# Sara-H-dev/Semantic_Segmentation_Of_StyleGAN2_Artifacts

Measured on AMD Instinct MI355X. Metric: training images/sec at 1024^2 bs=8 per GPU (MS-UNet Swin-T, fwd+DynamicLoss+bwd+AdamW), higher is better.
Workload: dtype bf16; 1 GPU; 1xMI355X 1024x1024 bs=8 Swin-T MS-UNet train step; model=MS-UNet swin_t, global_batch=8, world_size=1, img_size=1024, parallelism=dp1, grad_allreduce=f32, dead_branches=executed (no grad), step_execution=eager, params=42881040

## Files before the change

### include/msunet_hip.h

```cpp
#ifndef MSUNET_HIP_H
#define MSUNET_HIP_H

#ifdef __cplusplus
extern "C" {
#endif

int msu_layernorm_fwd(int dtype, int mode, const void* x, const void* b, const float* bscale,
                      long rows_per_sample, void* s_out, const float* gamma, const float* beta,
                      void* y, float* mean, float* rstd, long rows, int C, int H, int W, int Cin,
                      float eps, void* stream);
int msu_layernorm_bwd(int dtype, int mode, const void* dy, const void* x, const void* dres,
                      const float* gamma, const float* mean, const float* rstd, void* dx,
                      void* db, const float* bscale, long rows_per_sample, float* part,
                      int nparts, float* dgamma, float* dbeta, long rows, int C, int H, int W,
                      int Cin, int accumulate, void* stream);
int msu_layernorm_bwd3(int dtype, int mode, const void* dy, const void* x, const void* dres,
                       const void* dres2, const void* dres3, const float* gamma, const float* mean,
                       const float* rstd, void* dx, void* db, const float* bscale, long rows_per_sample,
                       float* part, int nparts, float* dgamma, float* dbeta, long rows, int C, int H, int W,
                       int Cin, int accumulate, void* stream);
int msu_ln_part_blocks(long rows, int C);
int msu_colsum_batch(int nseg, const float* const* part, const long* stride, const int* nparts, const int* n,
                     float* const* out, int accumulate, void* stream);
int msu_tail_reduce_mode(int mode);
// ... 46 lines not shown
int msu_conv3x3_wgrad(int dtype, int in_mode, const void* X, const void* dY, float* dW, float* db,
                      float* workspace, void* unused, int nchunk, int B, int H, int W, int Cin,
                      int Cout, void* stream);
int msu_conv3x3_wgrad2(int dtype, int in_mode, const void* X, const void* dY, float* dW, float* db,
                       float* workspace, int nchunk, int B, int H, int W, int Cin, int Cout, int accumulate,
                       void* stream);

int msu_win_attn_qkv_supported(int C, int nh);
int msu_win_attn_qkv_fwd(int dtype, const void* x, const void* w_qkv, const float* b_qkv, const float* table,
                         void* out, void* qkv_out, void* keep, float* workspace, int B, int H, int W, int C, int nh,
                         int shift, float p_drop, unsigned long long seed, const unsigned long long* seed_dev,
                         void* stream);
int msu_win_attn_qkv_fwd2(int dtype, const void* x, const void* w_qkv, const float* b_qkv, const float* table,
                          const void* w_proj, const float* b_proj, void* out, void* o_out, void* qkv_out, void* keep,
                          float* workspace, int B, int H, int W, int C, int nh, int shift, float p_drop,
                          unsigned long long seed, const unsigned long long* seed_dev, void* stream);

int msu_wgrad_splits(long M, int N, int K);
long msu_wgrad_workspace(long M, int N, int K);
int msu_linear_wgrad(int dtype, const void* dY, const void* X, float* dW, float* db, float* workspace,
                     long M, int N, int K, int accumulate, void* stream);
int msu_linear_wgrad_ld(int dtype, const void* dY, const void* X, float* dW, long ldw, float* db,
                        float* workspace, long M, int N, int K, int accumulate, void* stream);

int msu_linear_bwd_supported(long M, int K, int N);
long msu_linear_bwd_workspace(long M, int K, int N);
int msu_linear_bwd(int dtype, const void* dY, const void* X, const void* Wt, const void* H, void* dX, float* dW,
                   float* db, float* workspace, long M, int K, int N, int accumulate, void* stream);

int msu_tok_gemm_supported(long M, int N, int K);
int msu_tok_gemm_supported_epi(long M, int N, int K, int epi);
int msu_tok_gemm(int dtype, const void* A, const void* A2, int K1, const void* W, const float* bias, void* Y,
                 void* Y2, const void* H, long M, int N, int K, int epi, void* stream);
int msu_tok_gemm_plan(long M, int N, int K, long* out6);
int msu_nt_gemm_supported(long M, int N, int K);
int msu_nt_gemm_plan(long M, int N);
int msu_nt_gemm_mode(int mode);
int msu_nt_gemm(int dtype, const void* A, const void* W, const float* bias, void* Y, void* Y2, const void* H,
                long M, int N, int K, int epi, void* stream);
int msu_nt_gemm_cat(int dtype, const void* A, const void* A2, int K1, const void* W, const float* bias, void* Y,
                    long M, int N, int K, void* stream);
int msu_nt_gemm_kn(int dtype, const void* A, const void* Wk, const float* bias, void* Y, void* Y2, const void* H,
                   long M, int N, int K, int epi, void* stream);

int msu_mlp_fused_supported(int C, int Hd);
int msu_add_ln_mlp_fwd(int dtype, const void* a, const void* br, const float* bscale, long rows_per_sample,
// ... 64 lines not shown
```

### semantic_segmentation_of_stylegan2_artifacts_amd/_lib.py

```python
import ctypes
import os

from . import switches

_HERE = os.path.dirname(os.path.abspath(__file__))
LIB_PATH = switches.get("MSU_LIB_OVERRIDE") or os.path.join(_HERE, "libmsunet_hip.so")

P = ctypes.c_void_p
I = ctypes.c_int
L = ctypes.c_long
F = ctypes.c_float
D = ctypes.c_double
U64 = ctypes.c_ulonglong

SIGNATURES = {
    "msu_ln_part_blocks": (I, [L, I]),
    "msu_layernorm_fwd": (I, [I, I, P, P, P, L, P, P, P, P, P, P, L, I, I, I, I, F, P]),
    "msu_layernorm_bwd": (I, [I, I, P, P, P, P, P, P, P, P, P, L, P, I, P, P, L, I, I, I, I, I, P]),
    "msu_layernorm_bwd3": (I, [I, I, P, P, P, P, P, P, P, P, P, P, P, L, P, I, P, P, L, I, I, I, I, I, P]),
    "msu_reduce_rows": (I, [P, I, I, L, P, I, P]),
    "msu_tail_reduce_mode": (I, [I]),
    "msu_conv_mode": (I, [I]),
    "msu_head_fwd": (I, [I, P, P, P, P, P, P, P, L, I, F, P]),
    "msu_head_bwd": (I, [I, P, P, P, P, P, P, P, P, P, I, P, P, P, L, I, P]),
# ... 23 lines not shown
    "msu_dynloss_fwd2": (I, [I, P, P, I, L, F, F, F, P, I, P, P, P, P]),
    "msu_dynloss_fwd3": (I, [I, P, P, I, L, F, F, F, P, I, P, P, P, P, P]),
    "msu_dynloss_bwd2": (I, [I, P, P, P, P, P, I, L, F, F, F, P, P]),
    "msu_adamw": (I, [P, P, P, P, L, F, F, F, F, F, I, P, P, P]),
    "msu_nonfinite": (I, [P, L, P, P]),
    "msu_nonfinite2": (I, [P, L, P, L, P, P]),
    "msu_adamw_dev": (I, [P, P, P, P, L, P, D, D, D, D, P, P, P]),
    "msu_adamw_dev2": (I, [P, P, P, P, L, P, D, D, D, D, P, P, P, I, I, P]),
    "msu_step_advance": (I, [P, P, P]),
    "msu_cast": (I, [I, P, P, L, P]),
    "msu_colsum_batch": (I, [I, P, P, P, P, P, I, P]),
    "msu_conv3x3_weight": (I, [I, P, P, I, I, I, P]),
    "msu_transpose16_multi": (I, [P, P, P, I, I, P]),
    "msu_conv3x3_fwd": (I, [I, I, P, P, P, P, I, I, I, I, I, P]),
    "msu_conv3x3_fwd2": (I, [I, I, P, P, P, P, P, I, I, I, I, I, P]),
    "msu_conv3x3_dgrad": (I, [I, I, P, P, P, P, I, I, I, I, I, P]),
    "msu_conv3x3_wgrad_workspace": (L, [I, I, I, I, I]),
    "msu_conv3x3_wgrad": (I, [I, I, P, P, P, P, P, P, I, I, I, I, I, I, P]),
    "msu_conv3x3_wgrad2": (I, [I, I, P, P, P, P, P, I, I, I, I, I, I, I, P]),
    "msu_wgrad_splits": (I, [L, I, I]),
    "msu_wgrad_workspace": (L, [L, I, I]),
    "msu_linear_wgrad": (I, [I, P, P, P, P, P, L, I, I, I, P]),
    "msu_linear_wgrad_ld": (I, [I, P, P, P, L, P, P, L, I, I, I, P]),
    "msu_linear_bwd_supported": (I, [L, I, I]),
    "msu_linear_bwd_workspace": (L, [L, I, I]),
    "msu_linear_bwd": (I, [I, P, P, P, P, P, P, P, P, L, I, I, I, P]),
    "msu_tok_gemm_supported": (I, [L, I, I]),
    "msu_tok_gemm_supported_epi": (I, [L, I, I, I]),
    "msu_tok_gemm": (I, [I, P, P, I, P, P, P, P, P, L, I, I, I, P]),
    "msu_tok_gemm_plan": (I, [L, I, I, P]),
    "msu_nt_gemm_supported": (I, [L, I, I]),
    "msu_nt_gemm_plan": (I, [L, I]),
    "msu_nt_gemm_mode": (I, [I]),
    "msu_nt_gemm": (I, [I, P, P, P, P, P, P, L, I, I, I, P]),
    "msu_nt_gemm_kn": (I, [I, P, P, P, P, P, P, L, I, I, I, P]),
    "msu_nt_gemm_cat": (I, [I, P, P, I, P, P, P, L, I, I, P]),
    "msu_metrics_nblk": (I, [L]),
    "msu_seg_metrics": (I, [I, P, P, I, L, F, P, I, P, P]),
    "msu_augment_batch": (I, [P, P, P, P, P, P, I, I, I, P]),
    "msu_pred_maps_nblk": (I, [I, I]),
    "msu_pred_maps": (I, [I, P, P, P, I, I, I, F, F, F, F, I, I, P, P, P, P, P, P, P, P]),
}

_lib = None


# ... 35 lines not shown
```

### semantic_segmentation_of_stylegan2_artifacts_amd/csrc/common.h

```cpp
#pragma once
#include <hip/hip_runtime.h>
#include <hip/hip_bf16.h>
#include <stdint.h>

#include <mutex>

#define MSU_DEV __device__ __forceinline__

typedef __bf16 bf16x8 __attribute__((ext_vector_type(8)));
typedef float f32x4 __attribute__((ext_vector_type(4)));
typedef float f32x16 __attribute__((ext_vector_type(16)));
typedef uint32_t u32x4 __attribute__((ext_vector_type(4)));
typedef uint32_t u32x2 __attribute__((ext_vector_type(2)));
typedef float f32x2 __attribute__((ext_vector_type(2)));
typedef uint16_t bf16_t;
typedef _Float16 f16_t;
typedef _Float16 f16x8 __attribute__((ext_vector_type(8)));

enum MsuDtype { MSU_F32 = 0, MSU_BF16 = 1, MSU_F16 = 2 };

MSU_DEV float to_f32(float v) { return v; }
MSU_DEV float to_f32(bf16_t v) { return __uint_as_float(((uint32_t)v) << 16); }
template <typename T> MSU_DEV T from_f32(float v);
template <> MSU_DEV float from_f32<float>(float v) { return v; }
// ... 112 lines not shown
  const float cdf = 0.5f * (1.0f + erf_fast(x * 0.70710678118654752f, e));
  return fmaf(x * 0.39894228040143268f, e, cdf);
}

MSU_DEV f32x2 pk_fma(f32x2 a, f32x2 b, f32x2 c) { return __builtin_elementwise_fma(a, b, c); }
MSU_DEV f32x2 splat2(float v) { return f32x2{v, v}; }
MSU_DEV f32x2 erf_fast2(f32x2 x, f32x2& e_neg_x2) {
  const f32x2 ax = {fabsf(x.x), fabsf(x.y)};
  const f32x2 d = pk_fma(splat2(0.3275911f), ax, splat2(1.0f));
  const f32x2 t = {__builtin_amdgcn_rcpf(d.x), __builtin_amdgcn_rcpf(d.y)};
  f32x2 p = pk_fma(splat2(1.061405429f), t, splat2(-1.453152027f));
  p = pk_fma(p, t, splat2(1.421413741f));
  p = pk_fma(p, t, splat2(-0.284496736f));
  p = pk_fma(p, t, splat2(0.254829592f)) * t;
  const f32x2 q = -ax * ax;
  e_neg_x2 = f32x2{__expf(q.x), __expf(q.y)};
  const f32x2 r = pk_fma(-p, e_neg_x2, splat2(1.0f));
  return f32x2{copysignf(r.x, x.x), copysignf(r.y, x.y)};
}
MSU_DEV f32x2 gelu_fast2(f32x2 x) {
  f32x2 e;
  return splat2(0.5f) * x * (splat2(1.0f) + erf_fast2(x * splat2(0.70710678118654752f), e));
}

MSU_DEV float hash_uniform(uint64_t seed, uint64_t idx) {
  uint64_t z = seed + 0x9E3779B97F4A7C15ull * (idx + 1);
  z = (z ^ (z >> 30)) * 0xBF58476D1CE4E5B9ull;
  z = (z ^ (z >> 27)) * 0x94D049BB133111EBull;
  z ^= z >> 31;
  return (float)(uint32_t)(z >> 40) * (1.0f / 16777216.0f);
}

MSU_DEV uint64_t launch_seed(uint64_t seed, const unsigned long long* seed_dev) {
  if (seed_dev == nullptr) return seed;
  uint64_t z = seed ^ ((uint64_t)seed_dev[0] * 0x9E3779B97F4A7C15ull);
  z = (z ^ (z >> 31)) * 0xBF58476D1CE4E5B9ull;
  return z ^ (z >> 29);
}

MSU_DEV uint32_t fmix32_hash(uint32_t seed, uint32_t idx) {
  uint32_t x = idx * 0x9E3779B9u + seed;
  x ^= x >> 16; x *= 0x85EBCA6Bu;
  x ^= x >> 13; x *= 0xC2B2AE35u;
  return x ^ (x >> 16);
}
MSU_DEV uint32_t drop_thresh16(float p) { return (uint32_t)ceilf(p * 65536.0f); }
// ... 125 lines not shown
```

### semantic_segmentation_of_stylegan2_artifacts_amd/csrc/gemm_linbwd.hip

```cpp
#include <utility>

#include "common.h"
#include "reduce.h"

#ifndef MSU_EXP
#define MSU_EXP 0
#endif

namespace {

#ifndef MSU_LB_TS64
#define MSU_LB_TS64 1
#endif
constexpr int ts_of(int K, int N) { return (MSU_LB_TS64 && K == 96 && (N == 288 || N == 96)) ? 64 : 32; }
constexpr int NW = 8;
constexpr int NTHR = 64 * NW;

typedef short v4s __attribute__((ext_vector_type(4)));
typedef __attribute__((address_space(3))) v4s lds_v4s;

template <int I> using IC = std::integral_constant<int, I>;

template <typename F, int... I>
MSU_DEV __attribute__((always_inline)) void static_for_impl(F&& f, std::integer_sequence<int, I...>) {
// ... 82 lines not shown
MSU_DEV int wg_tile(int w, int i) {
  using P = Plan<K, N>;
  constexpr auto t = P::make();
  int jt = -1;
#pragma unroll
  for (int ww = 0; ww < NW; ++ww)
    if (w == ww && i < t.count[ww]) jt = t.tile[ww][i];
  return jt;
}

template <typename T, int K, int N, bool GG, bool GX = false>
__global__ void __launch_bounds__(NTHR, 1)
linbwd_kernel(const bf16_t* __restrict__ dY, const bf16_t* __restrict__ X, const bf16_t* __restrict__ Wt,
              const bf16_t* __restrict__ H, bf16_t* __restrict__ dX, float* __restrict__ part, long M) {
  using P = Plan<K, N>;
  constexpr int TM = ts_of(K, N);
  static_assert(!GG || TM == 32, "the GELU' operands are staged for 32-token steps");
  constexpr int LDW = N + 8, LDY = N + 8, LDX = ldx_of<K>();
  constexpr int CY = N / 8, CX = K / 8;
  constexpr int CHUNKS = TM * (CY + CX);
  constexpr int PER = (CHUNKS + NTHR - 1) / NTHR;
  constexpr int STAGE = TM * (LDY + LDX);
  constexpr int KT = P::KT, NS16 = P::NS16, DMAX = P::DMAX, WMAX = P::WMAX;
  extern __shared__ __attribute__((aligned(16))) unsigned char smem_raw[];
  bf16_t* sW = reinterpret_cast<bf16_t*>(smem_raw);
  bf16_t* sS = sW + K * LDW;
  const int tid = threadIdx.x, lane = tid & 63;
  const int wave = __builtin_amdgcn_readfirstlane(tid >> 6);
  const int h = lane >> 5;
  const long ntiles = (M + TM - 1) / TM;
  const int G = gridDim.x;
  const int b = blockIdx.x;
  const long nsteps = (ntiles - 1 - b) / G + 1;

  for (int i = tid; i < K * CY; i += NTHR) {
    const int r = i / CY, c = i - r * CY;
    *reinterpret_cast<u32x4*>(sW + r * LDW + 8 * c) = *reinterpret_cast<const u32x4*>(Wt + (long)r * N + 8 * c);
  }

  constexpr int D = ring_depth<K, N, GG>();
  u32x4 st[D][PER];
  int goff[PER], loff[PER];
#pragma unroll
  for (int j = 0; j < PER; ++j) {
    const int c = tid + NTHR * j;
    goff[j] = 0;
    loff[j] = 0;
    if (c < TM * CY) {
      const int r = c / CY, cc = c - r * CY;
      goff[j] = r * N + 8 * cc;
      loff[j] = r * LDY + 8 * cc;
    } else if (c < CHUNKS) {
      const int c2 = c - TM * CY;
      const int r = c2 / CX, cc = c2 - r * CX;
      goff[j] = r * K + 8 * cc;
      loff[j] = TM * LDY + r * LDX + 8 * cc;
    }
  }
  auto kind = [&](int j) __attribute__((always_inline)) {
    const int cw = wave * 64 + NTHR * j;
    return cw < TM * CY ? 0 : cw < CHUNKS ? 1 : 2;
  };
  auto load = [&](long step_, auto SET) __attribute__((always_inline)) {
    constexpr int set = decltype(SET)::value;
    const long step = step_ < nsteps ? step_ : nsteps - 1;
    const long m0 = (b + step * G) * TM;
    if (m0 + TM <= M) {
#pragma unroll
      for (int j = 0; j < PER; ++j) {
        const int kd = kind(j);
        const bf16_t* base = kd == 0 ? dY + m0 * N : kd == 1 ? X + m0 * K : dY;
        if constexpr ((MSU_EXP & 8) != 0) st[set][j] = u32x4{(unsigned)goff[j], 0u, 0u, 0u};
        else st[set][j] = gload16_s(base, 2u * (unsigned)goff[j]);
      }
    } else {
      const int t0 = opaque(tid);
#pragma unroll
      for (int j = 0; j < PER; ++j) {
        const int c = t0 + NTHR * j;
        const bf16_t* src = dY;
        if (c < TM * CY) {
          const int r = c / CY, cc = c - r * CY;
          const long m = m0 + r < M ? m0 + r : M - 1;
          src = dY + m * N + 8 * cc;
        } else if (c < CHUNKS) {
          const int c2 = c - TM * CY;
          const int r = c2 / CX, cc = c2 - r * CX;
          const long m = m0 + r < M ? m0 + r : M - 1;
          src = X + m * K + 8 * cc;
        }
        st[set][j] = gload16(src);
      }
    }
  };
  auto store = [&](long step, auto SET) __attribute__((always_inline)) {
    constexpr int set = decltype(SET)::value;
    if constexpr (GX) {
#pragma unroll
      for (int j = 0; j < PER; ++j) {
        if (kind(j) == 1) {
          u32x4& q = st[set][j];
#pragma unroll
          for (int i = 0; i < 4; ++i)
            q[i] = pack2<T>(gelu_fast(Fmt16<T>::lo(q[i])), gelu_fast(Fmt16<T>::hi(q[i])));
        }
      }
    }
    bf16_t* y = sS + (int)(step & 1) * STAGE;
    const long m0 = (b + step * G) * TM;
    if (m0 + TM <= M) {
#pragma unroll
      for (int j = 0; j < PER; ++j)
        if (kind(j) != 2) *reinterpret_cast<u32x4*>(y + loff[j]) = st[set][j];
    } else {
      const int t0 = opaque(tid);
#pragma unroll
      for (int j = 0; j < PER; ++j) {
        const int c = t0 + NTHR * j;
        const int r = c < TM * CY ? c / CY : (c - TM * CY) / CX;
        const u32x4 z = {0u, 0u, 0u, 0u};
        if (kind(j) != 2) *reinterpret_cast<u32x4*>(y + loff[j]) = m0 + r < M ? st[set][j] : z;
      }
    }
  };

  f32x16 accw[WMAX];
#pragma unroll
  for (int i = 0; i < WMAX; ++i) accw[i] = f32x16{0};
  constexpr int NP = N / 2, RG = NTHR / NP < TM ? NTHR / NP : TM;
  const int bp = tid % NP, bg = tid / NP;
  float db0 = 0.f, db1 = 0.f;

  static_for<D>([&](auto I) __attribute__((always_inline)) {
    load(decltype(I)::value, I);
  });
  store(0, IC<0>{});
  __syncthreads();

  auto body = [&](long s, auto SLOT) __attribute__((always_inline)) {
    constexpr int slot = decltype(SLOT)::value;
    const bf16_t* y = sS + (int)(s & 1) * STAGE;
    const bf16_t* x = y + TM * LDY;
    const long m0 = (b + s * G) * TM;
    u32x4 hv[DMAX][2];
    if constexpr (GG) {
      const long m = m0 + (lane & 31);
      const long mh = m < M ? m : M - 1;
#pragma unroll
      for (int d = 0; d < DMAX; ++d) {
        const int kt0 = wave + NW * d;
        if (MSU_LB_HALL || kt0 < KT) {
          const int kt = kt0 < KT ? kt0 : wave;
#pragma unroll
          for (int pp = 0; pp < 2; ++pp) hv[d][pp] = gload16(H + mh * K + 32 * kt + 16 * pp + 8 * h);
        }
      }
    }
    load(s + D, SLOT);

#pragma unroll
    for (int i = 0; i < WMAX; ++i) {
      const int jt = wg_tile<K, N>(wave, i);
      if (jt >= 0 && (MSU_EXP & 4) == 0) {
        const int jo = opaque(jt);
        const int kt = jo / P::NT, nt = jo - (jo / P::NT) * P::NT;
#pragma unroll
        for (int ks = 0; ks < TM / 16; ++ks)
          accw[i] = Fmt16<T>::mma32(frag_tr(x, LDX, 16 * ks, 32 * kt, lane), frag_tr(y, LDY, 16 * ks, 32 * nt, lane),
// ... 12 lines not shown

#pragma unroll
    for (int d = 0; d < DMAX; ++d) {
      const int kt = wave + NW * d;
#pragma unroll
      for (int tt = 0; tt < TM / 32; ++tt) if (kt < KT) {
        const long m = m0 + 32 * tt + (lane & 31);
        f32x16 acc = f32x16{0};
#pragma unroll 3
        for (int ns = 0; ns < ((MSU_EXP & 2) ? 0 : NS16); ++ns)
          acc = Fmt16<T>::mma32(frag_rows(sW, LDW, 32 * kt, 16 * ns, lane), frag_rows(y, LDY, 32 * tt, 16 * ns, lane),
                                acc);
#pragma unroll
        for (int pp = 0; pp < 2; ++pp) {
          const int g0 = 2 * pp;
          float v[8];
#pragma unroll
          for (int e = 0; e < 4; ++e) {
            const auto r = __builtin_amdgcn_permlane32_swap(__float_as_uint(acc[4 * g0 + e]),
                                                            __float_as_uint(acc[4 * g0 + 4 + e]), false, false);
            v[e] = __uint_as_float(r[0]);
            v[4 + e] = __uint_as_float(r[1]);
          }
          if constexpr (GG) {
#pragma unroll
            for (int e = 0; e < 4; ++e) {
              v[2 * e] *= gelu_grad_fast(Fmt16<T>::lo(hv[d][pp][e]));
              v[2 * e + 1] *= gelu_grad_fast(Fmt16<T>::hi(hv[d][pp][e]));
            }
          }
          const u32x4 pk = {pack2<T>(v[0], v[1]), pack2<T>(v[2], v[3]), pack2<T>(v[4], v[5]), pack2<T>(v[6], v[7])};
          if (m < M && (MSU_EXP & 1) == 0) *reinterpret_cast<u32x4*>(dX + m * K + 32 * kt + 16 * pp + 8 * h) = pk;
        }
      }
    }
    if (s + 1 < nsteps) {
      store(s + 1, IC<(slot + 1) % D>{});
    }
    __syncthreads();
  };
  for (long s = 0; s < nsteps; s += D) {
    static_for<D>([&](auto I) __attribute__((always_inline)) {
      if (s + decltype(I)::value < nsteps) body(s + decltype(I)::value, I);
    });
  }

  float* pw = part + (long)b * (N * K + N);
// ... 112 lines not shown
```

### semantic_segmentation_of_stylegan2_artifacts_amd/csrc/gemm_wgrad.hip

```cpp
#include <stdlib.h>

#include "common.h"
#include "mfma_frag.h"
#include "reduce.h"

#ifndef MSU_EXP
#define MSU_EXP 0
#endif

namespace {

constexpr int BM = 64;

MSU_DEV void unpack8(const u32x4& q, float (&v)[8]) {
#pragma unroll
  for (int i = 0; i < 4; ++i) {
    v[2 * i] = __uint_as_float(q[i] << 16);
    v[2 * i + 1] = __uint_as_float(q[i] & 0xffff0000u);
  }
}

template <typename T, int NTW>
__global__ void __launch_bounds__(256) wgrad_kernel(const T* __restrict__ dY, const T* __restrict__ X,
                                                    float* __restrict__ part, float* __restrict__ dbpart,
                                                    long M, int N, int K, long mchunk) {
  constexpr int WT = 16 * NTW;
  constexpr int BT = 2 * WT;
  constexpr int LDT = BT + 8;
  constexpr int EPC = 16 / (int)sizeof(T);
  constexpr int CPR = BT / EPC;
  constexpr int CH = BM * CPR / 256;
  __shared__ __attribute__((aligned(16))) T sA[2][BM * LDT];
  __shared__ __attribute__((aligned(16))) T sB[2][BM * LDT];
  const int tid = threadIdx.x, lane = tid & 63, wave = tid >> 6;
  const int ntk = (K + BT - 1) / BT;
  const int tn = blockIdx.x / ntk, tk = blockIdx.x - (blockIdx.x / ntk) * ntk;
  const int n0 = tn * BT, k0 = tk * BT;
  const long m_begin = (long)blockIdx.y * mchunk;
  long m_end = m_begin + mchunk;
  if (m_end > M) m_end = M;
  const int wn = (wave >> 1) * WT, wk = (wave & 1) * WT;

  f32x4 acc[NTW][NTW];
#pragma unroll
  for (int i = 0; i < NTW; ++i)
#pragma unroll
    for (int j = 0; j < NTW; ++j) acc[i][j] = f32x4{0.f, 0.f, 0.f, 0.f};
  float dbacc = 0.f;
  const bool do_bias = dbpart != nullptr && tk == 0;

  uint4 ra[CH], rb[CH];
  auto load_regs = [&](long m0) {
#pragma unroll
    for (int c = 0; c < CH; ++c) {
      const int idx = tid + 256 * c;
      const int r = idx / CPR, col = (idx - r * CPR) * EPC;
      const long m = m0 + r;
      const bool ok = m < m_end;
      ra[c] = (ok && n0 + col < N) ? *reinterpret_cast<const uint4*>(dY + m * (long)N + n0 + col) : make_uint4(0, 0, 0, 0);
      rb[c] = (ok && k0 + col < K) ? *reinterpret_cast<const uint4*>(X + m * (long)K + k0 + col) : make_uint4(0, 0, 0, 0);
    }
  };
  auto store_regs = [&](int buf) {
#pragma unroll
    for (int c = 0; c < CH; ++c) {
      const int idx = tid + 256 * c;
      const int r = idx / CPR, col = (idx - r * CPR) * EPC;
      *reinterpret_cast<uint4*>(&sA[buf][r * LDT + col]) = ra[c];
      *reinterpret_cast<uint4*>(&sB[buf][r * LDT + col]) = rb[c];
    }
  };

  int buf = 0;
  if (m_begin < m_end) {
    load_regs(m_begin);
    store_regs(0);
  }
  __syncthreads();
  for (long m0 = m_begin; m0 < m_end; m0 += BM) {
    const bool more = m0 + BM < m_end;
    if (more) load_regs(m0 + BM);
    const T* A = sA[buf];
    const T* B = sB[buf];
    auto rowA = [&](int k) { return A + k * LDT; };
    auto rowB = [&](int k) { return B + k * LDT; };
#pragma unroll
    for (int ks = 0; ks < BM; ks += 32)
#pragma unroll
      for (int i = 0; i < NTW; ++i)
#pragma unroll
        for (int j = 0; j < NTW; ++j) TR<T>::mma(acc[i][j], rowA, wn + 16 * i, rowB, wk + 16 * j, ks, lane);
// ... 1 lines not shown
#pragma unroll 8
      for (int r = 0; r < BM; ++r) dbacc += to_f32(A[r * LDT + tid]);
    }
    if (more) store_regs(buf ^ 1);
    __syncthreads();
    buf ^= 1;
  }
  float* out = part + (long)blockIdx.y * N * K;
#pragma unroll
  for (int i = 0; i < NTW; ++i)
#pragma unroll
    for (int j = 0; j < NTW; ++j)
#pragma unroll
      for (int r = 0; r < 4; ++r) {
        const int n = n0 + wn + 16 * i + (lane >> 4) * 4 + r;
        const int k = k0 + wk + 16 * j + (lane & 15);
        if (n < N && k < K) out[(long)n * K + k] = acc[i][j][r];
      }
  if (do_bias && tid < BT && n0 + tid < N) dbpart[(long)blockIdx.y * N + n0 + tid] = dbacc;
}

template <int WN, int WK> constexpr int wgrad_nw() { return WN * WK == 3 ? 3 : 4; }

template <typename T, int NTW, int WN, int WK, int NST>
__global__ void __launch_bounds__(256) wgrad_wave_kernel(const bf16_t* __restrict__ dY, const bf16_t* __restrict__ X,
                                                         float* __restrict__ part, float* __restrict__ dbpart,
                                                         long M, int N, int K, long mchunk, int ntiles) {
  constexpr int NW = wgrad_nw<WN, WK>();
  constexpr int WM = NW / (WN * WK), WT = 16 * NTW, BN = WN * WT, BK = WK * WT, RS = 32 * WM;
  static_assert(WM * WN * WK == NW, "wave split");
  constexpr int SA = (BN + 8) / 8, SB = (BK + 8) / 8;
  constexpr int LA = 8 * SA, LB = 8 * SB;
  constexpr int SLOTS = RS * (SA + SB);
  constexpr int INS = ((SLOTS + 63) / 64 + NW - 1) / NW * NW;
  constexpr int PER_WAVE = INS / NW;
  constexpr int STG = INS * 64 * 8;
  static_assert(NST >= 2 && PER_WAVE * (NST - 2) < 64, "vmcnt");
  extern __shared__ __attribute__((aligned(16))) unsigned char smem_raw[];
  bf16_t* lds = reinterpret_cast<bf16_t*>(smem_raw);
  const int tid = threadIdx.x, lane = tid & 63;
  const int wave = __builtin_amdgcn_readfirstlane(tid >> 6);
  const int wni = wave % WN, wki = (wave / WN) % WK, wmi = wave / (WN * WK);
  const int ntk = K / BK;
  const int item = xcd_remap(blockIdx.x, gridDim.x);
  const int split = item / ntiles, tile = item - split * ntiles;
  const int tn = tile / ntk, tk = tile - (tile / ntk) * ntk;
  const int n0 = tn * BN, k0 = tk * BK;
// ... 34 lines not shown
    }
  };

  f32x4 acc[NTW][NTW];
  f32x4 accb[NTW];
#pragma unroll
  for (int i = 0; i < NTW; ++i) {
    accb[i] = f32x4{0.f, 0.f, 0.f, 0.f};
#pragma unroll
    for (int j = 0; j < NTW; ++j) acc[i][j] = f32x4{0.f, 0.f, 0.f, 0.f};
  }
  const bool do_bias = dbpart != nullptr && tk == 0 && wki == 0;
  const bf16x8 ones = splat8<T>(1.0f, 1.0f, 1.0f);
  const int q = (lane & 15) >> 2, p4 = 4 * (lane & 3), r0 = wmi * 32 + 2 * (4 * ((lane >> 4) & 1) + q) + (lane >> 5);
  const int laneA = r0 * LA + wni * WT + p4, laneB = RS * LA + r0 * LB + wki * WT + p4;
  auto tr8 = [](const bf16_t* p, int second) {
    typedef __attribute__((address_space(3))) msu_v4s lds_v4s;
    const msu_v4s lo = __builtin_amdgcn_ds_read_tr16_b64_v4i16((lds_v4s*)(p));
    const msu_v4s hi = __builtin_amdgcn_ds_read_tr16_b64_v4i16((lds_v4s*)(p + second));
    msu_v4s both[2] = {lo, hi};
    return *reinterpret_cast<bf16x8*>(both);
  };

#pragma unroll
  for (int st = 0; st < NST - 1; ++st) issue(st);
  for (int st = 0; st < nstage; ++st) {
    wait_vmcnt<PER_WAVE * (NST - 2)>();
    __builtin_amdgcn_s_barrier();
    issue(st + NST - 1);
    if constexpr (MSU_EXP & 2) continue;
    const bf16_t* buf = lds + (st % NST) * STG;
    const uint32_t pa = lds_u32(buf + laneA), pb = lds_u32(buf + laneB);
    bf16x8 bf[NTW], af[2];
    unroll_for<NTW>([&](auto J) {
      constexpr int j = decltype(J)::value;
      bf[j] = tr8_untracked<32 * j, 32 * j + 32 * LB>(pb);
    });
    af[0] = tr8_untracked<0, 32 * LA>(pa);
    asm volatile("s_waitcnt lgkmcnt(0)" ::: "memory");
#pragma unroll
    for (int j = 0; j < NTW; ++j) asm volatile("" : "+v"(bf[j]));
    asm volatile("" : "+v"(af[0]));
    unroll_for<NTW>([&](auto I) {
      constexpr int i = decltype(I)::value;
      if constexpr (i + 1 < NTW) af[(i + 1) & 1] = tr8_untracked<32 * (i + 1), 32 * (i + 1) + 32 * LA>(pa);
#pragma unroll
      for (int j = 0; j < NTW; ++j) {
        if constexpr (MSU_EXP & 1)
          acc[i][j][0] += (float)af[i & 1][j] * (float)bf[j][i];
        else
          acc[i][j] = Fmt16<T>::mma16(af[i & 1], bf[j], acc[i][j]);
      }
// ... 94 lines not shown
  const int wt = 16 * p.ntw, nt = N / wt, kt = K / wt;
  pick_wave_split(nt, kt, p.wn, p.wk);
  const int nw = p.wn * p.wk == 3 ? 3 : 4;
  const int rs = 32 * (nw / (p.wn * p.wk));
  {
    const int sa = (p.wn * wt + 8) / 8, sb = (p.wk * wt + 8) / 8;
    const int ins = ((rs * (sa + sb) + 63) / 64 + nw - 1) / nw * nw;
    const int nst = (int)((160L * 1024) / ((long)ins * 64 * 16));
    if (nst < 3) {
      p.ntw = 0;
      return p;
    }
    p.nst = 3;
  }
  const long tiles = (long)(nt / p.wn) * (kt / p.wk);
  long s = ((MSU_EXP & 512) ? 128 : 256) / tiles;
  const long max_s = (M + 8 * rs - 1) / (8 * rs);
  if (s > max_s) s = max_s;
  if (s < 1) s = 1;
  p.S = (int)s;
  return p;
}

template <typename T, int NTW, int WN, int WK, int NST>
void launch_wave(dim3 grid, const bf16_t* dY, const bf16_t* X, float* part, float* dbpart, long M, int N, int K,
                 long mchunk, int ntiles, hipStream_t st) {
  constexpr int NW = wgrad_nw<WN, WK>();
  constexpr int WM = NW / (WN * WK), WT = 16 * NTW, RS = 32 * WM;
  constexpr int SLOTS = RS * ((WN * WT + 8) / 8 + (WK * WT + 8) / 8);
  constexpr int INS = ((SLOTS + 63) / 64 + NW - 1) / NW * NW;
  constexpr size_t lds = (size_t)NST * INS * 64 * 16;
  if constexpr (lds <= 160 * 1024) {
    auto kern = wgrad_wave_kernel<T, NTW, WN, WK, NST>;
    static bool attr_set = false;
    if (!attr_set) {
      (void)hipFuncSetAttribute((const void*)kern, hipFuncAttributeMaxDynamicSharedMemorySize, (int)lds);
      attr_set = true;
    }
    hipLaunchKernelGGL(kern, grid, dim3(64 * NW), lds, st, dY, X, part, dbpart, M, N, K, mchunk, ntiles);
  }
}

template <typename T>
int run_wave(const WavePlan& p, const bf16_t* dY, const bf16_t* X, float* part, float* dbpart, long M, int N, int K,
             hipStream_t st) {
  const int wt = 16 * p.ntw, nw = p.wn * p.wk == 3 ? 3 : 4, wm = nw / (p.wn * p.wk), rs = 32 * wm;
  long mchunk = (M + p.S - 1) / p.S;
  mchunk = (mchunk + rs - 1) / rs * rs;
  const int ntiles = (N / (p.wn * wt)) * (K / (p.wk * wt));
  const dim3 grid((unsigned)(ntiles * p.S));
#define MSU_WAVE(NTW, WN, WK)                                                                                        \
  if (p.ntw == NTW && p.wn == WN && p.wk == WK) {                                                                   \
    launch_wave<T, NTW, WN, WK, 3>(grid, dY, X, part, dbpart, M, N, K, mchunk, ntiles, st);                         \
    return 0;                                                                                                       \
  }
  MSU_WAVE(6, 1, 1) MSU_WAVE(6, 2, 1) MSU_WAVE(6, 4, 1) MSU_WAVE(6, 1, 2) MSU_WAVE(6, 2, 2) MSU_WAVE(6, 1, 4)
  MSU_WAVE(6, 3, 1) MSU_WAVE(6, 1, 3)
  MSU_WAVE(8, 1, 1) MSU_WAVE(8, 2, 1) MSU_WAVE(8, 4, 1) MSU_WAVE(8, 1, 2) MSU_WAVE(8, 2, 2) MSU_WAVE(8, 1, 4)
  MSU_WAVE(8, 3, 1) MSU_WAVE(8, 1, 3)
#undef MSU_WAVE
  return -3;
}

inline int tile_of(int N, int K) { return (N % 128 == 0 && K % 128 == 0) ? 128 : 96; }

inline int pick_splits(long M, int N, int K) {
  const int bt = tile_of(N, K);
  const long tiles = (long)((N + bt - 1) / bt) * ((K + bt - 1) / bt);
  long s = (1024 + tiles - 1) / tiles;
  const long max_s = (M + 511) / 512;
  if (s > max_s) s = max_s;
  if (s < 1) s = 1;
  return (int)s;
}

}

extern "C" {

int msu_wgrad_splits(long M, int N, int K) { return pick_splits(M, N, K); }

long msu_wgrad_workspace(long M, int N, int K) {
  const int S = pick_splits(M, N, K);
  long ws = (long)S * N * K + (long)S * N;
  const WavePlan p = wave_plan(M, N, K);
  if (p.ntw) {
    const long w2 = (long)p.slabs() * N * K + (long)p.slabs() * N;
    if (w2 > ws) ws = w2;
  }
  return ws;
}

int msu_linear_wgrad_ld(int dtype, const void* dY, const void* X, float* dW, long ldw, float* db,
                        float* workspace, long M, int N, int K, int accumulate, void* stream) {
  if (N % 8 || K % 8 || M < 0 || ldw < K) return -2;
  hipStream_t st = (hipStream_t)stream;
  if constexpr ((MSU_EXP & 256) != 0) return 0;
  if (M == 0) {
    if (!accumulate) hipMemset2DAsync(dW, sizeof(float) * ldw, 0, sizeof(float) * K, N, st);
    if (db && !accumulate) hipMemsetAsync(db, 0, sizeof(float) * N, st);
    return MSU_CHECK_LAUNCH();
  }
  if (msu_is16(dtype)) {
    const WavePlan p = wave_plan(M, N, K);
    if (p.ntw) {
      float* part = workspace;
      float* dbpart = db ? workspace + (long)p.slabs() * N * K : nullptr;
      int rc = -3;
      MSU_DISPATCH16(dtype, T, rc = run_wave<T>(p, (const bf16_t*)dY, (const bf16_t*)X, part, dbpart, M, N, K, st));
      if (rc) return rc;
      const ColSeg segs[2] = {{part, (long)N * K, (long)N * K, dW, K, ldw}, {dbpart, N, N, db}};
      colsum_multi(segs, db ? 2 : 1, p.slabs(), accumulate, st);
      return MSU_CHECK_LAUNCH();
    }
  }
  const int S = pick_splits(M, N, K);
  long mchunk = (M + S - 1) / S;
  mchunk = (mchunk + BM - 1) / BM * BM;
  float* part = workspace;
  float* dbpart = db ? workspace + (long)S * N * K : nullptr;
  const int bt = tile_of(N, K);
  const dim3 grid((unsigned)(((N + bt - 1) / bt) * ((K + bt - 1) / bt)), (unsigned)S);
  MSU_DISPATCH(dtype, T,
    if (bt == 96)
      hipLaunchKernelGGL((wgrad_kernel<T, 3>), grid, dim3(256), 0, st, (const T*)dY, (const T*)X, part, dbpart, M,
                         N, K, mchunk);
    else
      hipLaunchKernelGGL((wgrad_kernel<T, 4>), grid, dim3(256), 0, st, (const T*)dY, (const T*)X, part, dbpart, M,
                         N, K, mchunk));
  const ColSeg segs[2] = {{part, (long)N * K, (long)N * K, dW, K, ldw}, {dbpart, N, N, db}};
  colsum_multi(segs, db ? 2 : 1, S, accumulate, st);
  return MSU_CHECK_LAUNCH();
}

int msu_linear_wgrad(int dtype, const void* dY, const void* X, float* dW, float* db, float* workspace,
                     long M, int N, int K, int accumulate, void* stream) {
  return msu_linear_wgrad_ld(dtype, dY, X, dW, K, db, workspace, M, N, K, accumulate, stream);
}

}
```

### semantic_segmentation_of_stylegan2_artifacts_amd/csrc/mfma_frag.h

```cpp
#pragma once
#include <utility>

#include "common.h"

namespace {

typedef short msu_v4s __attribute__((ext_vector_type(4)));

template <typename T> struct TR;
template <typename T> struct TR16 {
  template <typename RowFn>
  static MSU_DEV bf16x8 frag(RowFn row_ptr, int kbase, int col0, int lane) {
    const int gq = lane >> 4, li = lane & 15, q = li >> 2, p = li & 3;
    const auto* a0 = row_ptr(kbase + 8 * gq + q) + col0 + 4 * p;
    const auto* a1 = row_ptr(kbase + 8 * gq + 4 + q) + col0 + 4 * p;
    typedef __attribute__((address_space(3))) msu_v4s lds_v4s;
    const msu_v4s lo = __builtin_amdgcn_ds_read_tr16_b64_v4i16((lds_v4s*)(a0));
    const msu_v4s hi = __builtin_amdgcn_ds_read_tr16_b64_v4i16((lds_v4s*)(a1));
    msu_v4s both[2] = {lo, hi};
    return *reinterpret_cast<bf16x8*>(both);
  }
  template <typename RA, typename RB>
  static MSU_DEV void mma(f32x4& acc, RA ra, int colA, RB rb, int colB, int kbase, int lane) {
    acc = Fmt16<T>::mma16(frag(ra, kbase, colA, lane), frag(rb, kbase, colB, lane), acc);
  }
};
template <> struct TR<bf16_t> : TR16<bf16_t> {};
template <> struct TR<f16_t> : TR16<f16_t> {};
template <int OFF>
MSU_DEV msu_v4s ds_tr_b64_untracked(uint32_t addr) {
  msu_v4s v;
  asm volatile("ds_read_b64_tr_b16 %0, %1 offset:%2" : "=v"(v) : "v"(addr), "i"(OFF));
  return v;
}
template <int OFF>
MSU_DEV uint32_t ds_b32_untracked(uint32_t addr) {
  uint32_t v;
  asm volatile("ds_read_b32 %0, %1 offset:%2" : "=v"(v) : "v"(addr), "i"(OFF));
  return v;
}
template <int OFF0, int OFF1>
MSU_DEV bf16x8 tr8_untracked(uint32_t addr) {
  const msu_v4s lo = ds_tr_b64_untracked<OFF0>(addr);
  const msu_v4s hi = ds_tr_b64_untracked<OFF1>(addr);
  return __builtin_bit_cast(bf16x8, __builtin_shufflevector(lo, hi, 0, 1, 2, 3, 4, 5, 6, 7));
}
template <typename T>
MSU_DEV void vreg_pin(T& v) {
  asm volatile("" : "+v"(v));
}
template <int N, typename... Fr>
MSU_DEV void lds_wait_tie(Fr&... fr) {
  static_assert(N >= 0 && N < 16, "lgkmcnt range");
  asm volatile("s_waitcnt lgkmcnt(%0)" : : "i"(N) : "memory");
  (vreg_pin(fr), ...);
}
template <typename F, int... Is>
MSU_DEV void unroll_for_impl(F&& f, std::integer_sequence<int, Is...>) {
  (f(std::integral_constant<int, Is>{}), ...);
}
template <int N, typename F>
MSU_DEV void unroll_for(F&& f) {
  unroll_for_impl(f, std::make_integer_sequence<int, N>{});
// ... 18 lines not shown
```

### semantic_segmentation_of_stylegan2_artifacts_amd/ops.py

```python
import contextlib
import ctypes
import functools

import torch

from . import _lib, switches

_DT = {torch.float32: 0, torch.bfloat16: 1, torch.float16: 2}
_LOW = (torch.bfloat16, torch.float16)


def _dt(t):
    try:
        return _DT[t.dtype]
    except KeyError:
        raise TypeError(f"unsupported activation dtype {t.dtype} (float32 / bfloat16 / float16)") from None


def _need_cuda(*ts):
    for t in ts:
        if t is not None and not t.is_cuda:
            raise RuntimeError("msunet HIP ops need tensors on a HIP device (no CPU fallback)")


# ... 783 lines not shown
    _lib.call("msu_nt_gemm_kn", _dt(a), _p(a), _p(wk), None, _p(y), None, _p(h), M, N, K, epi, _s(a))
    return y


def _wt(w):
    return w.t().contiguous()


def _gemm_dx(dy, w, epi=TOK_PLAIN, h=None, param=None):
    N, K = w.shape
    M = dy.numel() // N
    wt = _shadow_t(param, w.dtype)
    if gemm_route(M, K, N, epi) == "nt" and wt is None:
        return nt_gemm_kn(dy, w, epi, h)
    return _gemm(dy, _wt(w) if wt is None else wt, None, epi, h)


def _gelu16(h):
    g = torch.empty_like(h)
    _lib.call("msu_gelu_fwd", _dt(h), _p(h), _p(g), h.numel(), _s(h))
    return g


def _wgrad_launch(dy, x, dw, db, M, N, K, acc, x_gelu_of=None):
    if x is None:
        x = _gelu16(x_gelu_of)
    ws = torch.empty(_lib.lib().msu_wgrad_workspace(M, N, K), device=x.device, dtype=torch.float32)
    _lib.call("msu_linear_wgrad_ld", _dt(x), _p(dy), _p(x), _p(dw), dw.stride(0), _p(db), _p(ws), M, N, K, acc,
              _s(x))


def _wgrad(dy, x, weight, bias, M, N, K, x_gelu_of=None, side_ok=True):
    src = x if x is not None else x_gelu_of
    if not (_direct(weight) and (bias is None or _direct(bias))):
        dw = torch.empty(N, K, device=src.device, dtype=torch.float32)
        db = torch.empty(N, device=src.device, dtype=torch.float32) if bias is not None else None
        _wgrad_launch(dy, x, dw, db, M, N, K, 0, x_gelu_of)
        return dw, db
    side = _side_enabled and _side_wgrad and side_ok
    with _on_side(src.device, (dy, src), (weight, bias)) if side else contextlib.nullcontext():
        _wgrad_launch(dy, x, weight.grad, None if bias is None else bias.grad, M, N, K, 1, x_gelu_of)
    if not side:
        _notify(weight, bias)
    return None, None


def _shadow(param, dt):
    sh = getattr(param, "_msu_shadow", None)
    if sh is not None and sh.dtype == dt and getattr(param, "_msu_shadow_ver", -1) == param._version:
        return sh
    return param.to(dt)

# ... 925 lines not shown
```

Baseline: 179.5 images/s.

## Fuse GELU recompute into weight-gradient GEMM staging instead of a separate kernel

```diff
diff --git a/include/msunet_hip.h b/include/msunet_hip.h
--- a/include/msunet_hip.h
+++ b/include/msunet_hip.h
@@ -92,6 +92,8 @@
                      long M, int N, int K, int accumulate, void* stream);
 int msu_linear_wgrad_ld(int dtype, const void* dY, const void* X, float* dW, long ldw, float* db,
                         float* workspace, long M, int N, int K, int accumulate, void* stream);
+int msu_linear_wgrad_ld_gelu(int dtype, const void* dY, const void* H, float* dW, long ldw, float* db,
+                             float* workspace, long M, int N, int K, int accumulate, void* stream);
 
 int msu_linear_bwd_supported(long M, int K, int N);
 long msu_linear_bwd_workspace(long M, int K, int N);
diff --git a/semantic_segmentation_of_stylegan2_artifacts_amd/_lib.py b/semantic_segmentation_of_stylegan2_artifacts_amd/_lib.py
--- a/semantic_segmentation_of_stylegan2_artifacts_amd/_lib.py
+++ b/semantic_segmentation_of_stylegan2_artifacts_amd/_lib.py
@@ -69,6 +69,7 @@
     "msu_wgrad_workspace": (L, [L, I, I]),
     "msu_linear_wgrad": (I, [I, P, P, P, P, P, L, I, I, I, P]),
     "msu_linear_wgrad_ld": (I, [I, P, P, P, L, P, P, L, I, I, I, P]),
+    "msu_linear_wgrad_ld_gelu": (I, [I, P, P, P, L, P, P, L, I, I, I, P]),
     "msu_linear_bwd_supported": (I, [L, I, I]),
     "msu_linear_bwd_workspace": (L, [L, I, I]),
     "msu_linear_bwd": (I, [I, P, P, P, P, P, P, P, P, L, I, I, I, P]),
diff --git a/semantic_segmentation_of_stylegan2_artifacts_amd/csrc/common.h b/semantic_segmentation_of_stylegan2_artifacts_amd/csrc/common.h
--- a/semantic_segmentation_of_stylegan2_artifacts_amd/csrc/common.h
+++ b/semantic_segmentation_of_stylegan2_artifacts_amd/csrc/common.h
@@ -158,6 +158,23 @@
   f32x2 e;
   return splat2(0.5f) * x * (splat2(1.0f) + erf_fast2(x * splat2(0.70710678118654752f), e));
 }
+MSU_DEV void gelu_and_grad2(f32x2 x, f32x2& g, f32x2& dg) {
+  f32x2 e;
+  const f32x2 one_erf = splat2(1.0f) + erf_fast2(x * splat2(0.70710678118654752f), e);
+  g = splat2(0.5f) * x * one_erf;
+  dg = pk_fma(x * splat2(0.39894228040143268f), e, splat2(0.5f) * one_erf);
+}
+typedef __bf16 msu_bf16x2 __attribute__((ext_vector_type(2)));
+template <typename T> MSU_DEV uint32_t pack2v(f32x2 v) { return pack2<T>(v.x, v.y); }
+template <> MSU_DEV uint32_t pack2v<bf16_t>(f32x2 v) {
+  return __builtin_bit_cast(uint32_t, __builtin_convertvector(v, msu_bf16x2));
+}
+template <typename T> MSU_DEV u32x4 gelu8_pk(const u32x4& q) {
+  u32x4 o;
+#pragma unroll
+  for (int i = 0; i < 4; ++i) o[i] = pack2v<T>(gelu_fast2(f32x2{Fmt16<T>::lo(q[i]), Fmt16<T>::hi(q[i])}));
+  return o;
+}
 
 MSU_DEV float hash_uniform(uint64_t seed, uint64_t idx) {
   uint64_t z = seed + 0x9E3779B97F4A7C15ull * (idx + 1);
diff --git a/semantic_segmentation_of_stylegan2_artifacts_amd/csrc/gemm_linbwd.hip b/semantic_segmentation_of_stylegan2_artifacts_amd/csrc/gemm_linbwd.hip
--- a/semantic_segmentation_of_stylegan2_artifacts_amd/csrc/gemm_linbwd.hip
+++ b/semantic_segmentation_of_stylegan2_artifacts_amd/csrc/gemm_linbwd.hip
@@ -128,6 +128,7 @@
   constexpr int PER = (CHUNKS + NTHR - 1) / NTHR;
   constexpr int STAGE = TM * (LDY + LDX);
   constexpr int KT = P::KT, NS16 = P::NS16, DMAX = P::DMAX, WMAX = P::WMAX;
+  static_assert(!GX || (GG && KT == 12 && DMAX == 2 && PER == 4 && NTHR / 2 * 2 >= TM * CY), "GX chunk deal");
   extern __shared__ __attribute__((aligned(16))) unsigned char smem_raw[];
   bf16_t* sW = reinterpret_cast<bf16_t*>(smem_raw);
   bf16_t* sS = sW + K * LDW;
@@ -146,13 +147,39 @@
 
   constexpr int D = ring_depth<K, N, GG>();
   u32x4 st[D][PER];
+  float gp[GX ? PER : 1][8];
+  auto gx_chunk = [&](int t, int j, int& r, int& col) __attribute__((always_inline)) {
+    const int w = t >> 6, l = t & 63;
+    r = 0;
+    col = 0;
+    if (w < KT - NW || j < 2) {
+      r = l & 31;
+      col = 32 * (w + NW * (j >> 1)) + 16 * (j & 1) + 8 * (l >> 5);
+      return 1;
+    }
+    const int c2 = (t - NTHR / 2) + NTHR / 2 * (j - 2);
+    if (c2 >= TM * CY) return 2;
+    r = c2 / CY;
+    col = 8 * (c2 - r * CY);
+    return 0;
+  };
   int goff[PER], loff[PER];
 #pragma unroll
   for (int j = 0; j < PER; ++j) {
     const int c = tid + NTHR * j;
     goff[j] = 0;
     loff[j] = 0;
-    if (c < TM * CY) {
+    if constexpr (GX) {
+      int r, col;
+      const int kd = gx_chunk(tid, j, r, col);
+      if (kd == 0) {
+        goff[j] = r * N + col;
+        loff[j] = r * LDY + col;
+      } else if (kd == 1) {
+        goff[j] = r * K + col;
+        loff[j] = TM * LDY + r * LDX + col;
+      }
+    } else if (c < TM * CY) {
       const int r = c / CY, cc = c - r * CY;
       goff[j] = r * N + 8 * cc;
       loff[j] = r * LDY + 8 * cc;
@@ -165,6 +192,7 @@
   }
   auto kind = [&](int j) __attribute__((always_inline)) {
     const int cw = wave * 64 + NTHR * j;
+    if constexpr (GX) return (wave < KT - NW || j < 2) ? 1 : (wave * 64 - NTHR / 2) + NTHR / 2 * (j - 2) < TM * CY ? 0 : 2;
     return cw < TM * CY ? 0 : cw < CHUNKS ? 1 : 2;
   };
   auto load = [&](long step_, auto SET) __attribute__((always_inline)) {
@@ -185,7 +213,12 @@
       for (int j = 0; j < PER; ++j) {
         const int c = t0 + NTHR * j;
         const bf16_t* src = dY;
-        if (c < TM * CY) {
+        if constexpr (GX) {
+          int r, col;
+          const int kd = gx_chunk(t0, j, r, col);
+          const long m = m0 + r < M ? m0 + r : M - 1;
+          if (kd != 2) src = (kd == 0 ? dY + m * N : X + m * K) + col;
+        } else if (c < TM * CY) {
           const int r = c / CY, cc = c - r * CY;
           const long m = m0 + r < M ? m0 + r : M - 1;
           src = dY + m * N + 8 * cc;
@@ -207,8 +240,13 @@
         if (kind(j) == 1) {
           u32x4& q = st[set][j];
 #pragma unroll
-          for (int i = 0; i < 4; ++i)
-            q[i] = pack2<T>(gelu_fast(Fmt16<T>::lo(q[i])), gelu_fast(Fmt16<T>::hi(q[i])));
+          for (int i = 0; i < 4; ++i) {
+            f32x2 g, dg;
+            gelu_and_grad2(f32x2{Fmt16<T>::lo(q[i]), Fmt16<T>::hi(q[i])}, g, dg);
+            q[i] = pack2v<T>(g);
+            gp[j][2 * i] = dg.x;
+            gp[j][2 * i + 1] = dg.y;
+          }
         }
       }
     }
@@ -223,7 +261,11 @@
 #pragma unroll
       for (int j = 0; j < PER; ++j) {
         const int c = t0 + NTHR * j;
-        const int r = c < TM * CY ? c / CY : (c - TM * CY) / CX;
+        int r = c < TM * CY ? c / CY : (c - TM * CY) / CX;
+        if constexpr (GX) {
+          int col;
+          gx_chunk(t0, j, r, col);
+        }
         const u32x4 z = {0u, 0u, 0u, 0u};
         if (kind(j) != 2) *reinterpret_cast<u32x4*>(y + loff[j]) = m0 + r < M ? st[set][j] : z;
       }
@@ -249,7 +291,7 @@
     const bf16_t* x = y + TM * LDY;
     const long m0 = (b + s * G) * TM;
     u32x4 hv[DMAX][2];
-    if constexpr (GG) {
+    if constexpr (GG && !GX) {
       const long m = m0 + (lane & 31);
       const long mh = m < M ? m : M - 1;
 #pragma unroll
@@ -308,7 +350,10 @@
             v[e] = __uint_as_float(r[0]);
             v[4 + e] = __uint_as_float(r[1]);
           }
-          if constexpr (GG) {
+          if constexpr (GX) {
+#pragma unroll
+            for (int e = 0; e < 8; ++e) v[e] *= gp[2 * d + pp][e];
+          } else if constexpr (GG) {
 #pragma unroll
             for (int e = 0; e < 4; ++e) {
               v[2 * e] *= gelu_grad_fast(Fmt16<T>::lo(hv[d][pp][e]));
diff --git a/semantic_segmentation_of_stylegan2_artifacts_amd/csrc/gemm_wgrad.hip b/semantic_segmentation_of_stylegan2_artifacts_amd/csrc/gemm_wgrad.hip
--- a/semantic_segmentation_of_stylegan2_artifacts_amd/csrc/gemm_wgrad.hip
+++ b/semantic_segmentation_of_stylegan2_artifacts_amd/csrc/gemm_wgrad.hip
@@ -20,7 +20,7 @@
   }
 }
 
-template <typename T, int NTW>
+template <typename T, int NTW, bool GX = false>
 __global__ void __launch_bounds__(256) wgrad_kernel(const T* __restrict__ dY, const T* __restrict__ X,
                                                     float* __restrict__ part, float* __restrict__ dbpart,
                                                     long M, int N, int K, long mchunk) {
@@ -67,6 +67,11 @@
       const int idx = tid + 256 * c;
       const int r = idx / CPR, col = (idx - r * CPR) * EPC;
       *reinterpret_cast<uint4*>(&sA[buf][r * LDT + col]) = ra[c];
+      if constexpr (GX) {
+        static_assert(sizeof(T) == 2, "GELU staging: 16-bit formats");
+        const u32x4 g = gelu8_pk<T>(u32x4{rb[c].x, rb[c].y, rb[c].z, rb[c].w});
+        rb[c] = make_uint4(g[0], g[1], g[2], g[3]);
+      }
       *reinterpret_cast<uint4*>(&sB[buf][r * LDT + col]) = rb[c];
     }
   };
@@ -114,7 +119,7 @@
 
 template <int WN, int WK> constexpr int wgrad_nw() { return WN * WK == 3 ? 3 : 4; }
 
-template <typename T, int NTW, int WN, int WK, int NST>
+template <typename T, int NTW, int WN, int WK, int NST, bool GX = false>
 __global__ void __launch_bounds__(256) wgrad_wave_kernel(const bf16_t* __restrict__ dY, const bf16_t* __restrict__ X,
                                                          float* __restrict__ part, float* __restrict__ dbpart,
                                                          long M, int N, int K, long mchunk, int ntiles) {
@@ -195,12 +200,41 @@
     return *reinterpret_cast<bf16x8*>(both);
   };
 
+  constexpr int CB = BK / 8, XCH = RS * CB, CPL = (XCH + 64 * NW - 1) / (64 * NW);
+  int goff[GX ? CPL : 1];
+  if constexpr (GX) {
+#pragma unroll
+    for (int i = 0; i < CPL; ++i) {
+      const int idx = tid + 64 * NW * i;
+      goff[i] = idx < XCH ? 2 * (RS * LA + (idx / CB) * LB + 8 * (idx % CB)) : -1;
+    }
+  }
+  auto gelu_stage = [&](int st) __attribute__((always_inline)) {
+    const uint32_t base = lds_u32(lds + (st % NST) * STG);
+    u32x4 v[CPL];
+#pragma unroll
+    for (int i = 0; i < CPL; ++i)
+      if ((i + 1) * 64 * NW <= XCH || goff[i] >= 0) v[i] = ds_chunk_untracked(base + goff[i]);
+    asm volatile("s_waitcnt lgkmcnt(0)" ::: "memory");
+#pragma unroll
+    for (int i = 0; i < CPL; ++i)
+      if ((i + 1) * 64 * NW <= XCH || goff[i] >= 0) {
+        vreg_pin(v[i]);
+        ds_chunk_write_untracked(base + goff[i], gelu8_pk<T>(v[i]));
+      }
+    asm volatile("s_waitcnt lgkmcnt(0)" ::: "memory");
+  };
+
 #pragma unroll
   for (int st = 0; st < NST - 1; ++st) issue(st);
   for (int st = 0; st < nstage; ++st) {
     wait_vmcnt<PER_WAVE * (NST - 2)>();
     __builtin_amdgcn_s_barrier();
     issue(st + NST - 1);
+    if constexpr (GX) {
+      gelu_stage(st);
+      __builtin_amdgcn_s_barrier();
+    }
     if constexpr (MSU_EXP & 2) continue;
     const bf16_t* buf = lds + (st % NST) * STG;
     const uint32_t pa = lds_u32(buf + laneA), pb = lds_u32(buf + laneB);
@@ -341,7 +375,7 @@
   return p;
 }
 
-template <typename T, int NTW, int WN, int WK, int NST>
+template <typename T, int NTW, int WN, int WK, int NST, bool GX>
 void launch_wave(dim3 grid, const bf16_t* dY, const bf16_t* X, float* part, float* dbpart, long M, int N, int K,
                  long mchunk, int ntiles, hipStream_t st) {
   constexpr int NW = wgrad_nw<WN, WK>();
@@ -350,7 +384,7 @@
   constexpr int INS = ((SLOTS + 63) / 64 + NW - 1) / NW * NW;
   constexpr size_t lds = (size_t)NST * INS * 64 * 16;
   if constexpr (lds <= 160 * 1024) {
-    auto kern = wgrad_wave_kernel<T, NTW, WN, WK, NST>;
+    auto kern = wgrad_wave_kernel<T, NTW, WN, WK, NST, GX>;
     static bool attr_set = false;
     if (!attr_set) {
       (void)hipFuncSetAttribute((const void*)kern, hipFuncAttributeMaxDynamicSharedMemorySize, (int)lds);
@@ -360,7 +394,7 @@
   }
 }
 
-template <typename T>
+template <typename T, bool GX>
 int run_wave(const WavePlan& p, const bf16_t* dY, const bf16_t* X, float* part, float* dbpart, long M, int N, int K,
              hipStream_t st) {
   const int wt = 16 * p.ntw, nw = p.wn * p.wk == 3 ? 3 : 4, wm = nw / (p.wn * p.wk), rs = 32 * wm;
@@ -370,7 +404,7 @@
   const dim3 grid((unsigned)(ntiles * p.S));
 #define MSU_WAVE(NTW, WN, WK)                                                                                        \
   if (p.ntw == NTW && p.wn == WN && p.wk == WK) {                                                                   \
-    launch_wave<T, NTW, WN, WK, 3>(grid, dY, X, part, dbpart, M, N, K, mchunk, ntiles, st);                         \
+    launch_wave<T, NTW, WN, WK, 3, GX>(grid, dY, X, part, dbpart, M, N, K, mchunk, ntiles, st);                         \
     return 0;                                                                                                       \
   }
   MSU_WAVE(6, 1, 1) MSU_WAVE(6, 2, 1) MSU_WAVE(6, 4, 1) MSU_WAVE(6, 1, 2) MSU_WAVE(6, 2, 2) MSU_WAVE(6, 1, 4)
@@ -410,8 +444,13 @@
   return ws;
 }
 
-int msu_linear_wgrad_ld(int dtype, const void* dY, const void* X, float* dW, long ldw, float* db,
-                        float* workspace, long M, int N, int K, int accumulate, void* stream) {
+}
+
+namespace {
+
+template <bool GX>
+int wgrad_ld(int dtype, const void* dY, const void* X, float* dW, long ldw, float* db, float* workspace, long M,
+             int N, int K, int accumulate, void* stream) {
   if (N % 8 || K % 8 || M < 0 || ldw < K) return -2;
   hipStream_t st = (hipStream_t)stream;
   if constexpr ((MSU_EXP & 256) != 0) return 0;
@@ -426,7 +465,7 @@
       float* part = workspace;
       float* dbpart = db ? workspace + (long)p.slabs() * N * K : nullptr;
       int rc = -3;
-      MSU_DISPATCH16(dtype, T, rc = run_wave<T>(p, (const bf16_t*)dY, (const bf16_t*)X, part, dbpart, M, N, K, st));
+      MSU_DISPATCH16(dtype, T, rc = (run_wave<T, GX>(p, (const bf16_t*)dY, (const bf16_t*)X, part, dbpart, M, N, K, st)));
       if (rc) return rc;
       const ColSeg segs[2] = {{part, (long)N * K, (long)N * K, dW, K, ldw}, {dbpart, N, N, db}};
       colsum_multi(segs, db ? 2 : 1, p.slabs(), accumulate, st);
@@ -440,18 +479,40 @@
   float* dbpart = db ? workspace + (long)S * N * K : nullptr;
   const int bt = tile_of(N, K);
   const dim3 grid((unsigned)(((N + bt - 1) / bt) * ((K + bt - 1) / bt)), (unsigned)S);
-  MSU_DISPATCH(dtype, T,
-    if (bt == 96)
-      hipLaunchKernelGGL((wgrad_kernel<T, 3>), grid, dim3(256), 0, st, (const T*)dY, (const T*)X, part, dbpart, M,
-                         N, K, mchunk);
-    else
-      hipLaunchKernelGGL((wgrad_kernel<T, 4>), grid, dim3(256), 0, st, (const T*)dY, (const T*)X, part, dbpart, M,
-                         N, K, mchunk));
+#define MSU_WGRAD_GENERIC(DISPATCH)                                                                                 \
+  DISPATCH(dtype, T,                                                                                               \
+    if (bt == 96)                                                                                                  \
+      hipLaunchKernelGGL((wgrad_kernel<T, 3, GX>), grid, dim3(256), 0, st, (const T*)dY, (const T*)X, part, dbpart, \
+                         M, N, K, mchunk);                                                                         \
+    else                                                                                                           \
+      hipLaunchKernelGGL((wgrad_kernel<T, 4, GX>), grid, dim3(256), 0, st, (const T*)dY, (const T*)X, part, dbpart, \
+                         M, N, K, mchunk))
+  if constexpr (GX) {
+    MSU_WGRAD_GENERIC(MSU_DISPATCH16);
+  } else {
+    MSU_WGRAD_GENERIC(MSU_DISPATCH);
+  }
+#undef MSU_WGRAD_GENERIC
   const ColSeg segs[2] = {{part, (long)N * K, (long)N * K, dW, K, ldw}, {dbpart, N, N, db}};
   colsum_multi(segs, db ? 2 : 1, S, accumulate, st);
   return MSU_CHECK_LAUNCH();
 }
 
+}
+
+extern "C" {
+
+int msu_linear_wgrad_ld(int dtype, const void* dY, const void* X, float* dW, long ldw, float* db,
+                        float* workspace, long M, int N, int K, int accumulate, void* stream) {
+  return wgrad_ld<false>(dtype, dY, X, dW, ldw, db, workspace, M, N, K, accumulate, stream);
+}
+
+int msu_linear_wgrad_ld_gelu(int dtype, const void* dY, const void* H, float* dW, long ldw, float* db,
+                             float* workspace, long M, int N, int K, int accumulate, void* stream) {
+  if (!msu_is16(dtype)) return -3;
+  return wgrad_ld<true>(dtype, dY, H, dW, ldw, db, workspace, M, N, K, accumulate, stream);
+}
+
 int msu_linear_wgrad(int dtype, const void* dY, const void* X, float* dW, float* db, float* workspace,
                      long M, int N, int K, int accumulate, void* stream) {
   return msu_linear_wgrad_ld(dtype, dY, X, dW, K, db, workspace, M, N, K, accumulate, stream);
diff --git a/semantic_segmentation_of_stylegan2_artifacts_amd/csrc/mfma_frag.h b/semantic_segmentation_of_stylegan2_artifacts_amd/csrc/mfma_frag.h
--- a/semantic_segmentation_of_stylegan2_artifacts_amd/csrc/mfma_frag.h
+++ b/semantic_segmentation_of_stylegan2_artifacts_amd/csrc/mfma_frag.h
@@ -39,6 +39,14 @@
   asm volatile("ds_read_b32 %0, %1 offset:%2" : "=v"(v) : "v"(addr), "i"(OFF));
   return v;
 }
+MSU_DEV u32x4 ds_chunk_untracked(uint32_t addr) {
+  u32x4 v;
+  asm volatile("ds_read_b128 %0, %1" : "=v"(v) : "v"(addr));
+  return v;
+}
+MSU_DEV void ds_chunk_write_untracked(uint32_t addr, const u32x4& v) {
+  asm volatile("ds_write_b128 %0, %1" : : "v"(addr), "v"(v) : "memory");
+}
 template <int OFF0, int OFF1>
 MSU_DEV bf16x8 tr8_untracked(uint32_t addr) {
   const msu_v4s lo = ds_tr_b64_untracked<OFF0>(addr);
diff --git a/semantic_segmentation_of_stylegan2_artifacts_amd/ops.py b/semantic_segmentation_of_stylegan2_artifacts_amd/ops.py
--- a/semantic_segmentation_of_stylegan2_artifacts_amd/ops.py
+++ b/semantic_segmentation_of_stylegan2_artifacts_amd/ops.py
@@ -829,12 +829,20 @@
     return g
 
 
+wgrad_gelu_calls = 0
+
+
 def _wgrad_launch(dy, x, dw, db, M, N, K, acc, x_gelu_of=None):
+    global wgrad_gelu_calls
+    entry = "msu_linear_wgrad_ld"
     if x is None:
-        x = _gelu16(x_gelu_of)
+        if x_gelu_of.dtype in _LOW:
+            x, entry = x_gelu_of.contiguous(), "msu_linear_wgrad_ld_gelu"
+            wgrad_gelu_calls += 1
+        else:
+            x = _gelu16(x_gelu_of)
     ws = torch.empty(_lib.lib().msu_wgrad_workspace(M, N, K), device=x.device, dtype=torch.float32)
-    _lib.call("msu_linear_wgrad_ld", _dt(x), _p(dy), _p(x), _p(dw), dw.stride(0), _p(db), _p(ws), M, N, K, acc,
-              _s(x))
+    _lib.call(entry, _dt(x), _p(dy), _p(x), _p(dw), dw.stride(0), _p(db), _p(ws), M, N, K, acc, _s(x))
 
 
 def _wgrad(dy, x, weight, bias, M, N, K, x_gelu_of=None, side_ok=True):
```

Result: no change. 181.2 images/s, median of 6 (+0.9%).
